# PKU-EPIC/GraspNeRF

Hardware: AMD Instinct MI355X
Metric: scenes/sec TSDF+render fwd, 6-view 40^3 grid (higher is better)
Workload: dtype f32

## Files before the change

graspnerf_amd/_lib.py:

```python
import ctypes as C
import os

_HERE = os.path.dirname(os.path.abspath(__file__))
LIB_PATH = os.path.join(_HERE, 'csrc', os.environ.get('GNR_LIB', 'libgnr.so'))

GNR_OK, GNR_ERR_ARG, GNR_ERR_SHAPE, GNR_ERR_HIP, GNR_ERR_WORKSPACE = 0, -1, -2, -3, -4
ERRORS = {-1: 'GNR_ERR_ARG', -2: 'GNR_ERR_SHAPE', -3: 'GNR_ERR_HIP', -4: 'GNR_ERR_WORKSPACE'}

c_float_p = C.POINTER(C.c_float)


class GnrScene(C.Structure):
    _fields_ = [('B', C.c_int), ('V', C.c_int), ('H', C.c_int), ('W', C.c_int), ('fh', C.c_int), ('fw', C.c_int),
                ('imgs', C.c_void_p), ('img_feats', C.c_void_p), ('ray_feats', C.c_void_p),
                ('poses', C.c_void_p), ('Ks', C.c_void_p), ('depth_range', C.c_void_p), ('use_vis', C.c_int), ('options', C.c_uint)]


OPTIONS = {'fp32_chain': 0x001, 'feature_grad_fixed': 0x002, 'view1_one_wavefront': 0x004, 'view2_one_wavefront': 0x008,
           'ray_order_morton': 0x010, 'poison_partials': 0x020, 'direct_scatter': 0x040, 'geo_dual_fp32': 0x080, 'test_lose_partner': 0x100, 'static_tiles': 0x200, 'split_launch': 0x400}
GNR_STATUS_LOST_PARTNER = 16


class GnrRays(C.Structure):
    _fields_ = [('rn', C.c_int), ('dn', C.c_int), ('fdn', C.c_int),
                ('ray_mask_view_num', C.c_int), ('ray_mask_point_num', C.c_int),
                ('coords', C.c_void_p), ('que_pose', C.c_void_p), ('que_K', C.c_void_p),
                ('que_depth_range', C.c_void_p), ('que_imgs', C.c_void_p), ('fine_u', C.c_void_p),
                ('ray_batch_num', C.c_int), ('fine_depth_use_all', C.c_int)]


RENDER_OUT_FIELDS = ['depth', 'sdf_values', 'alpha_values', 'colors_nr', 'hit_prob_nr', 'pixel_colors_nr',
                     'pixel_colors_gt', 'render_depth', 'ray_mask', 'sdf_gradient_error', 'sdf_gradient', 'view_mask']


class GnrRenderOut(C.Structure):
    _fields_ = [(k, C.c_void_p) for k in RENDER_OUT_FIELDS]


GNR_GAUSS_MAX_RADIUS = 16


class GnrSelectParams(C.Structure):
    _fields_ = [('gauss_radius', C.c_int), ('gauss_w', C.c_double * (GNR_GAUSS_MAX_RADIUS + 1)),
                ('tsdf_thres_high', C.c_float), ('tsdf_thres_low', C.c_float), ('min_width', C.c_float),
                ('max_width', C.c_float), ('threshold', C.c_float), ('dilate_iterations', C.c_int),
                ('max_filter_size', C.c_int)]


class GnrError(RuntimeError):
    pass


# ... 1 lines not shown


def lib():
    global _lib
    if _lib is not None:
        return _lib
    if not os.path.exists(LIB_PATH):
        raise GnrError(f'{LIB_PATH} not found: build it with graspnerf_amd/csrc/build.sh '
                       f'(or __graft_entry__.build()); there is no CPU fallback for the hot path')
    import torch
    L = C.CDLL(LIB_PATH)
    L.gnr_canonical_weights_floats.restype = C.c_int
    L.gnr_packed_weights_floats.restype = C.c_int
    L.gnr_pack_weights.argtypes = [c_float_p, c_float_p]
    L.gnr_pack_weights.restype = C.c_int
    L.gnr_pack_vis_decoder.argtypes = [c_float_p, c_float_p]
    L.gnr_pack_vis_decoder.restype = C.c_int
    L.gnr_pack_vis_decoder_bwd.argtypes = [c_float_p, c_float_p]
    L.gnr_pack_vis_decoder_bwd.restype = C.c_int
    L.gnr_canonical_vis_floats.restype = C.c_int
    for name in ('gnr_pack_weights_device', 'gnr_pack_weights_bwd_device', 'gnr_pack_vis_decoder_device', 'gnr_pack_vis_decoder_bwd_device'):
        getattr(L, name).argtypes = [C.c_void_p, C.c_void_p, C.c_void_p]
        getattr(L, name).restype = C.c_int
    L.gnr_layout_offset.argtypes = [C.c_char_p]
    L.gnr_layout_offset.restype = C.c_int
    L.gnr_workspace_bytes.argtypes = [C.POINTER(GnrScene), C.c_int, C.c_int, C.c_int]
    L.gnr_workspace_bytes.restype = C.c_size_t
    L.gnr_prepare.argtypes = [C.POINTER(GnrScene), C.c_void_p, C.c_size_t, C.c_void_p]
    L.gnr_prepare.restype = C.c_int
    L.gnr_range_status.argtypes = [C.POINTER(GnrScene), C.c_void_p, C.c_size_t, C.POINTER(C.c_uint), C.c_void_p]
    L.gnr_range_status.restype = C.c_int
    L.gnr_status_words_offset.argtypes = [C.POINTER(GnrScene)]
    L.gnr_status_words_offset.restype = C.c_size_t
    L.gnr_sample_volume_fwd.argtypes = [C.POINTER(GnrScene), C.c_void_p, C.c_int, C.c_void_p, C.c_void_p,
                                        C.c_void_p, C.c_void_p, C.c_size_t, C.c_void_p]
    L.gnr_sample_volume_fwd.restype = C.c_int
    L.gnr_debug_volume_chain.argtypes = [C.POINTER(GnrScene), C.c_void_p, C.c_int, C.c_void_p, C.c_void_p,
                                         C.c_void_p, C.c_size_t, C.c_void_p]
    L.gnr_debug_volume_chain.restype = C.c_int
    L.gnr_depth_mean_fwd.argtypes = [C.POINTER(GnrScene), C.c_void_p, C.c_int, C.c_void_p, C.c_void_p,
                                     C.c_void_p, C.c_size_t, C.c_void_p]
    L.gnr_depth_mean_fwd.restype = C.c_int
    L.gnr_merge_depths.argtypes = [C.c_void_p, C.c_int, C.c_void_p, C.c_int, C.c_void_p, C.c_int, C.c_void_p]
    L.gnr_merge_depths.restype = C.c_int
    L.gnr_render_by_depth_fwd.argtypes = [C.POINTER(GnrScene), C.POINTER(GnrRays), C.c_void_p, C.c_int, C.c_void_p,
                                          C.POINTER(GnrRenderOut), C.c_void_p, C.c_size_t, C.c_void_p]
    L.gnr_render_by_depth_fwd.restype = C.c_int
    L.gnr_render_rays_fwd.argtypes = [C.POINTER(GnrScene), C.POINTER(GnrRays), C.c_void_p, C.c_void_p,
                                      C.POINTER(GnrRenderOut), C.POINTER(GnrRenderOut), C.c_void_p, C.c_void_p,
                                      C.c_void_p, C.c_size_t, C.c_void_p]
    L.gnr_render_rays_fwd.restype = C.c_int
    L.gnr_head_canonical_floats.restype = C.c_int
    L.gnr_head_packed_floats.restype = C.c_int
    L.gnr_pack_grasp_head.argtypes = [c_float_p, c_float_p]
    L.gnr_pack_grasp_head.restype = C.c_int
    L.gnr_grasp_head_workspace_bytes.argtypes = [C.c_int, C.c_int]
    L.gnr_grasp_head_workspace_bytes.restype = C.c_size_t
    L.gnr_grasp_head_fwd.argtypes = [C.c_int, C.c_int, C.c_void_p, C.c_void_p, C.c_void_p, C.c_void_p, C.c_void_p,
                                     C.c_void_p, C.c_size_t, C.c_void_p]
    L.gnr_grasp_head_fwd.restype = C.c_int
    L.gnr_head_last_error.restype = C.c_char_p
    L.gnr_conv3d_bwd_weight.argtypes = [C.c_void_p] * 3 + [C.c_int] * 7 + [C.c_void_p]
    L.gnr_conv3d_same_bwd_weight.argtypes = [C.c_void_p] * 3 + [C.c_int] * 7 + [C.c_void_p, C.c_size_t, C.c_void_p]
    L.gnr_conv3d_same_bwd_weight_workspace_bytes.argtypes = [C.c_int] * 7
    L.gnr_conv3d_same_bwd_weight_workspace_bytes.restype = C.c_size_t
    L.gnr_conv3d_same_bwd_weight.restype = C.c_int
# ... 65 lines not shown
                                      [C.c_void_p] * 6 + [C.c_int, C.c_void_p, C.c_size_t, C.c_void_p]
    L.gnr_grasp_select_fwd.restype = C.c_int
    L.gnr_post_last_error.restype = C.c_char_p
    L.gnr_time_chain_kernel.argtypes = [C.POINTER(GnrScene), C.c_int, C.c_void_p, C.c_void_p, C.c_size_t, C.c_int,
                                        c_float_p, C.c_void_p]
    L.gnr_time_chain_kernel.restype = C.c_int
    L.gnr_chain_timing_begin.restype = C.c_int
    L.gnr_timing_begin.restype = C.c_int
    L.gnr_timing_begin_only.argtypes = [C.c_char_p]
    L.gnr_timing_begin_only.restype = C.c_int
    L.gnr_timing_end.argtypes = [C.c_char_p, C.c_size_t]
    L.gnr_timing_end.restype = C.c_int
    L.gnr_chain_timing_end.argtypes = [c_float_p, C.POINTER(C.c_int)]
    L.gnr_chain_timing_end.restype = C.c_int
    L.gnr_img_last_error.restype = C.c_char_p
    L.gnr_instnorm_act.argtypes = [C.c_void_p] * 7 + [C.c_longlong, C.c_int, C.c_int, C.c_float, C.c_int, C.c_void_p]
    L.gnr_instnorm_act.restype = C.c_int
    L.gnr_instnorm_act_bwd.argtypes = [C.c_void_p] * 12 + [C.c_longlong, C.c_int, C.c_int, C.c_int, C.c_void_p]
    L.gnr_instnorm_act_bwd.restype = C.c_int
    for fn in (L.gnr_reflect_pad2d, L.gnr_reflect_pad2d_bwd):
        fn.argtypes = [C.c_void_p, C.c_void_p, C.c_longlong, C.c_int, C.c_int, C.c_int, C.c_void_p]
        fn.restype = C.c_int
    L.gnr_upsample2x_bilinear.argtypes = [C.c_void_p, C.c_void_p, C.c_longlong, C.c_int, C.c_int, C.c_void_p]
    L.gnr_upsample2x_bilinear.restype = C.c_int
    L.gnr_last_error.restype = C.c_char_p
    L.gnr_dominant_kernel_name.restype = C.c_char_p
    L.gnr_debug_fill_lds.argtypes = [C.c_uint, C.c_void_p]
    L.gnr_debug_fill_lds.restype = C.c_int
    _lib = L
    return L


EXPORTED = ['gnr_canonical_weights_floats', 'gnr_packed_weights_floats', 'gnr_pack_weights', 'gnr_pack_vis_decoder', 'gnr_pack_vis_decoder_bwd', 'gnr_canonical_vis_floats', 'gnr_pack_weights_device', 'gnr_pack_weights_bwd_device', 'gnr_pack_vis_decoder_device', 'gnr_pack_vis_decoder_bwd_device', 'gnr_layout_offset', 'gnr_workspace_bytes',
            'gnr_prepare', 'gnr_range_status', 'gnr_status_words_offset', 'gnr_sample_volume_fwd', 'gnr_debug_volume_chain', 'gnr_depth_mean_fwd', 'gnr_merge_depths', 'gnr_render_by_depth_fwd', 'gnr_render_rays_fwd',
            'gnr_dominant_kernel_name', 'gnr_last_error', 'gnr_time_chain_kernel', 'gnr_head_canonical_floats',
            'gnr_head_packed_floats', 'gnr_pack_grasp_head', 'gnr_grasp_head_workspace_bytes', 'gnr_grasp_head_fwd',
            'gnr_head_last_error', 'gnr_chain_timing_begin', 'gnr_chain_timing_end', 'gnr_timing_begin', 'gnr_timing_begin_only', 'gnr_timing_end', 'gnr_grasp_select_workspace_bytes',
            'gnr_grasp_select_fwd', 'gnr_post_last_error', 'gnr_packed_bwd_floats', 'gnr_pack_weights_bwd',
            'gnr_depth_mean_bwd_workspace_bytes', 'gnr_depth_mean_bwd', 'gnr_sample_volume_train_workspace_bytes',
            'gnr_train_workspace_layout', 'gnr_sample_volume_fwd_train', 'gnr_sample_volume_bwd',
            'gnr_render_chain_train_workspace_bytes', 'gnr_render_chain_fwd_train', 'gnr_render_chain_bwd', 'gnr_conv3d_bwd_weight', 'gnr_conv3d_same_workspace_bytes', 'gnr_conv3d_same', 'gnr_conv3d_tap_mask_words', 'gnr_conv3d_tap_mask', 'gnr_conv3d_same_masked', 'gnr_conv3d_same_bwd_weight_masked', 'gnr_conv3d_same_bwd_weight', 'gnr_conv3d_same_bwd_weight_workspace_bytes',
            'gnr_render_tail_fwd_train', 'gnr_ray_tail_grad_floats', 'gnr_ray_tail_dual_bwd', 'gnr_ray_tail_dual_bwd_workspace_bytes', 'gnr_composite_bwd', 'gnr_composite_bwd_workspace_bytes', 'gnr_geo_dual_fwd', 'gnr_geo_dual_fwd_workspace_bytes', 'gnr_geo_dual_bwd', 'gnr_geo_dual_bwd_workspace_bytes', 'gnr_host_randperm_prefix',
            'gnr_debug_fill_lds', 'gnr_img_last_error', 'gnr_instnorm_act', 'gnr_instnorm_act_bwd', 'gnr_reflect_pad2d', 'gnr_reflect_pad2d_bwd', 'gnr_upsample2x_bilinear']


def check(rc, what):
    if rc != GNR_OK:
        msg = lib().gnr_last_error().decode(errors='replace')
        raise GnrError(f'{what} failed: {ERRORS.get(rc, rc)} ({msg})')


def timing_begin(only=None):
    check(lib().gnr_timing_begin_only(only.encode() if only else None), 'gnr_timing_begin')


def timing_end():
    buf = C.create_string_buffer(1 << 16)
    n = lib().gnr_timing_end(buf, len(buf))
    if n < 0:
        check(n, 'gnr_timing_end')
    out = {}
    for line in buf.value.decode().splitlines():
        label, cnt, ms = line.rsplit(' ', 2)
        out[label] = (int(cnt), float(ms))
    return out
```

graspnerf_amd/csrc/gnr_capi.inc:

```
#include <stdio.h>
#include <string.h>
#include <atomic>
#include <mutex>

#include "../../include/gnr.h"

namespace gnr {

static thread_local char g_err[512] = "";
static int fail(int code, const char* what, hipError_t e = hipSuccess) {
    snprintf(g_err, sizeof(g_err), "%s%s%s", what, e != hipSuccess ? ": " : "", e != hipSuccess ? hipGetErrorString(e) : "");
    return code;
}
#define GNR_HIP(call)                                                         \
    do {                                                                      \
        hipError_t e_ = (call);                                               \
        if (e_ != hipSuccess) return fail(GNR_ERR_HIP, #call, e_);            \
    } while (0)

static inline size_t al256(size_t x) { return (x + 255) & ~(size_t)255; }

static bool attr_needed(std::atomic<unsigned long long>& done) {
    int dev = 0;
    if (hipGetDevice(&dev) != hipSuccess) return true;
    const unsigned long long bit = 1ull << (dev & 63);
    if (done.load() & bit) return false;
    done.fetch_or(bit);
    return true;
}

struct Workspace {
    float* feat64; float* viewp; unsigned* range_flag;
    float* desc; float* rec; float* depth_c; float* depth_f; float* depth_m; float* gerr_part; unsigned char* vmask_pts;
    int* ray_perm;
    size_t total;
};

static Workspace carve(const GnrScene* s, size_t P, size_t rn, void* base) {
    Workspace w;
    char* p = (char*)base;
    size_t off = 0;
    const size_t BV = (size_t)s->B * s->V;
    auto take = [&](size_t bytes) { char* q = p ? p + off : nullptr; off += al256(bytes); return q; };
    w.feat64 = (float*)take(BV * s->fh * s->fw * 64 * sizeof(float));
    w.viewp = (float*)take(BV * VIEWP_FLOATS * sizeof(float));
    w.range_flag = (unsigned*)take(512);
    w.desc = (float*)take((size_t)s->B * P * DESC_FLOATS * sizeof(float));
    w.rec = (float*)take((size_t)s->B * P * REC_RAY * sizeof(float));
    w.depth_c = (float*)take((size_t)s->B * P * sizeof(float));
    w.depth_f = (float*)take((size_t)s->B * P * sizeof(float));
    w.depth_m = (float*)take((size_t)s->B * P * sizeof(float));
    w.gerr_part = (float*)take((size_t)s->B * (rn > 0 ? rn : 1) * sizeof(float));
    w.vmask_pts = (unsigned char*)take((size_t)s->B * P);
    w.ray_perm = (int*)take((size_t)s->B * (rn > 0 ? rn : 1) * sizeof(int));
    w.total = off;
    return w;
}

enum StatusSlot { RS_SCENE = 0, RS_VOLUME = 1, RS_COARSE = 2, RS_FINE = 3, RS_VOLUME_TRAIN = 4, RS_COARSE_TRAIN = 5, RS_DEPTHS_TRAIN = 6,
                  RS_BACKWARD = 61 , RS_RAY_WATCH = 62 ,
                  RS_FEAT_FX = 63 , RS_WORDS = 64 };
static_assert(RS_DEPTHS_TRAIN < RS_BACKWARD && RS_FEAT_FX < RS_WORDS, "status slots");
static inline bool opt(const GnrScene* s, unsigned bit) { return (s->options & bit) != 0; }

static int check_scene(const GnrScene* s) {
    if (!s || !s->imgs || !s->img_feats || !s->ray_feats || !s->poses || !s->Ks || !s->depth_range)
        return fail(GNR_ERR_ARG, "GnrScene: null pointer");
    if (s->options & ~GNR_OPT_ALL) return fail(GNR_ERR_ARG, "GnrScene.options: unknown bits (GNR_OPT_*)");
    if (s->B < 1 || s->H < 2 || s->W < 2 || s->fh < 1 || s->fw < 1) return fail(GNR_ERR_SHAPE, "GnrScene: bad dims");
    if (s->V < 2 || s->V > 8) return fail(GNR_ERR_SHAPE, "GnrScene: V must be in 2..8");
    return GNR_OK;
}

static int check_points(const GnrScene* s, size_t P) {
    if ((size_t)s->B * P > ((size_t)1 << 31) - 1024) return fail(GNR_ERR_SHAPE, "too many points in one call (B*P must stay below 2^31): split the rays / scenes");
    return GNR_OK;
}

static bool brick_order_ok(int R) { return R % 8 == 0; }

static int num_cus() {
    static int n = 0;
    if (!n) {
        hipDeviceProp_t prop;
        int dev = 0;
        if (hipGetDevice(&dev) != hipSuccess || hipGetDeviceProperties(&prop, dev) != hipSuccess) return 256;
        n = prop.multiProcessorCount > 0 ? prop.multiProcessorCount : 256;
// ... 315 lines not shown
    if (int rc = check_scene(s)) return rc;
    if (!ws) return fail(GNR_ERR_ARG, "workspace is null");
    Workspace w = carve(s, 0, 0, ws);
    if (ws_bytes < w.total) return fail(GNR_ERR_WORKSPACE, "workspace too small");
    hipStream_t st = (hipStream_t)stream;
    const int npix = s->fh * s->fw, BV = s->B * s->V;
    { KScope ks("k_view_setup@gnr_prepare", st); hipLaunchKernelGGL(k_view_setup, dim3((BV + 63) / 64), dim3(64), 0, st, s->poses, s->Ks, s->depth_range, w.viewp, BV, w.range_flag); }
    GNR_HIP(hipGetLastError());
    { KScope ks("k_repack_feats@gnr_prepare", st); hipLaunchKernelGGL(k_repack_feats, dim3((npix + 63) / 64, BV), dim3(256), 0, st, s->ray_feats, s->img_feats, w.feat64, npix, w.range_flag); }
    GNR_HIP(hipGetLastError());
    return GNR_OK;
}

extern "C" int gnr_range_status(const GnrScene* s, const void* ws, size_t ws_bytes, unsigned* flags_out, void* stream) {
    if (int rc = check_scene(s)) return rc;
    if (!ws || !flags_out) return fail(GNR_ERR_ARG, "gnr_range_status: null pointer");
    Workspace w = carve(s, 0, 0, const_cast<void*>(ws));
    if (ws_bytes < w.total) return fail(GNR_ERR_WORKSPACE, "workspace too small");
    hipStream_t st = (hipStream_t)stream;
    unsigned words[RS_WORDS];
    GNR_HIP(hipMemcpyAsync(words, w.range_flag, sizeof(words), hipMemcpyDeviceToHost, st));
    GNR_HIP(hipStreamSynchronize(st));
    unsigned f = 0;
    for (int i = 0; i < RS_WORDS; ++i) f |= words[i];
    *flags_out = f;
    return GNR_OK;
}

extern "C" size_t gnr_status_words_offset(const GnrScene* s) {
    if (!s) return 0;
    char* const base = (char*)4096;
    Workspace w = carve(s, 0, 0, base);
    return (size_t)((char*)w.range_flag - base);
}

struct SideStream { hipStream_t st = nullptr; hipEvent_t fork = nullptr, join = nullptr; };
static SideStream* side_stream() {
    static SideStream tab[64];
    static std::atomic<unsigned long long> made{0};
    int dev = 0;
    if (hipGetDevice(&dev) != hipSuccess) return nullptr;
    SideStream& e = tab[dev & 63];
    const unsigned long long bit = 1ull << (dev & 63);
    if (!(made.load() & bit)) {
        static std::mutex mu;
        std::lock_guard<std::mutex> lk(mu);
        if (!(made.load() & bit)) {
            if (hipStreamCreateWithFlags(&e.st, hipStreamNonBlocking) != hipSuccess) return nullptr;
            if (hipEventCreateWithFlags(&e.fork, hipEventDisableTiming) != hipSuccess || hipEventCreateWithFlags(&e.join, hipEventDisableTiming) != hipSuccess) return nullptr;
            made.fetch_or(bit);
        }
    }
    return &e;
}

static int volume_impl(const GnrScene* s, const float* bbox_min, int R, const float* wc, float* sdf_out,
                       unsigned char* vmask_out, void* ws, size_t ws_bytes, hipStream_t st, bool points, bool chain, bool ray,
                       float* dbg = nullptr) {
    if (int rc = check_points(s, (size_t)R * R * R)) return rc;
    Workspace w = carve(s, (size_t)R * R * R, 0, ws);
    if (ws_bytes < w.total) return fail(GNR_ERR_WORKSPACE, "workspace too small");
    const int P = R * R * R;
    const bool inline_pts = GNR_VOLUME_POINTS_INLINE != 0 && chain && ray && !dbg && R * R * R < (1 << 22);
    if (points && !inline_pts) {
        { KScope ks("k_points_volume@volume_impl", st); hipLaunchKernelGGL(k_points_volume, dim3((s->B * P + 255) / 256), dim3(256), 0, st, bbox_min, w.desc, R, s->B); }
        GNR_HIP(hipGetLastError());
// ... 25 lines not shown
            if (int rc = launch_ray<false>(r, ps)) return rc;
        }
    }
    if (split) { GNR_HIP(hipEventRecord(side->join, side->st)); GNR_HIP(hipStreamWaitEvent(st, side->join, 0)); }
    return GNR_OK;
}

extern "C" int gnr_sample_volume_fwd(const GnrScene* s, const float* bbox_min, int R, const float* wc, float* sdf_out,
                                     unsigned char* vmask_out, void* ws, size_t ws_bytes, void* stream) {
    if (int rc = check_scene(s)) return rc;
    if (!bbox_min || !wc || !sdf_out || !ws) return fail(GNR_ERR_ARG, "gnr_sample_volume_fwd: null pointer");
    if (R < 2 || R > MAX_DN) return fail(GNR_ERR_SHAPE, "volume_res must be in 2..64");
    return volume_impl(s, bbox_min, R, wc, sdf_out, vmask_out, ws, ws_bytes, (hipStream_t)stream, true, true, true);
}

extern "C" int gnr_debug_volume_chain(const GnrScene* s, const float* bbox_min, int R, const float* wc, float* dbg,
                                      void* ws, size_t ws_bytes, void* stream) {
    if (int rc = check_scene(s)) return rc;
    if (!bbox_min || !wc || !dbg || !ws) return fail(GNR_ERR_ARG, "gnr_debug_volume_chain: null pointer");
    return volume_impl(s, bbox_min, R, wc, nullptr, nullptr, ws, ws_bytes, (hipStream_t)stream, true, true, false, dbg);
}

static int order_rays(const GnrScene* s, const GnrRays* q, Workspace& w, hipStream_t st, const int** perm_out) {
    *perm_out = nullptr;
    if (!opt(s, GNR_OPT_RAY_ORDER_MORTON) || q->rn > MAX_SORT_RAYS || q->rn < 2) return GNR_OK;
    int shift = 0;
    while (((s->W > s->H ? s->W : s->H) >> shift) > 1024) ++shift;
    { KScope ks("k_ray_order@render_pass", st); hipLaunchKernelGGL(k_ray_order, dim3(s->B), dim3(256), 0, st, q->coords, w.ray_perm, q->rn, shift); }
    GNR_HIP(hipGetLastError());
    *perm_out = w.ray_perm;
    return GNR_OK;
}

static int render_pass(const GnrScene* s, const GnrRays* q, const float* depth, int dn, const float* wl, GnrRenderOut* out,
                       Workspace& w, hipStream_t st, float* fine_depth, int* fine_inds, int fdn, const float* fine_u = nullptr,
                       const int* perm = nullptr, int range_slot = RS_COARSE, float* gt_also = nullptr, bool skip_gt = false, bool gen_depth = false) {
    if (!out || !out->colors_nr) return fail(GNR_ERR_ARG, "GnrRenderOut.colors_nr is required");
    const int B = s->B, rn = q->rn;
    const int P = rn * dn;
    { KScope ks("k_points_rays@render_pass", st); hipLaunchKernelGGL(k_points_rays, dim3((B * P + 255) / 256), dim3(256), 0, st, q->coords, q->que_pose, q->que_K,
                       q->que_depth_range, depth, w.desc, rn, dn, B, perm, gen_depth ? const_cast<float*>(depth) : nullptr); }
    GNR_HIP(hipGetLastError());
    ChainArgs a{wl, w.feat64, s->imgs, w.viewp, w.desc, w.rec, out->colors_nr, out->view_mask, nullptr,
                B, P, s->H, s->W, s->fh, s->fw, 0};
    a.range_flag = w.range_flag;
    a.range_launch = w.range_flag ? w.range_flag + range_slot : nullptr;
    a.tile_ctr = (w.range_flag && !opt(s, GNR_OPT_STATIC_TILES)) ? w.range_flag + RS_WORDS : nullptr;
    a.ray_perm = perm; a.perm_rn = rn; a.perm_dn = dn;
    if (int rc = launch_chain<true>(s, a, st)) return rc;
    RayArgs r;
    memset(&r, 0, sizeof(r));
    r.wpk = wl; r.rec = w.rec; r.desc = w.desc; r.depth = depth; r.colors = out->colors_nr; r.que_dr = q->que_depth_range;
    r.nrays = B * rn; r.dn = dn; r.rays_per_scene = rn;
    r.sdf = out->sdf_values; r.alpha = out->alpha_values; r.hit = out->hit_prob_nr; r.pix = out->pixel_colors_nr;
    r.rdepth = out->render_depth; r.gerr_part = out->sdf_gradient_error ? w.gerr_part : nullptr; r.grad = out->sdf_gradient;
    r.rmask = out->ray_mask; r.view_num = q->ray_mask_view_num; r.point_num = q->ray_mask_point_num;
    r.fine_depth = fine_depth; r.fine_inds = fine_inds; r.fdn = fdn; r.fine_u = fine_u; r.ray_perm = perm;
    r.range_word = w.range_flag ? w.range_flag + RS_RAY_WATCH : nullptr;
    if (int rc = launch_ray<true>(r, st)) return rc;
    if (out->sdf_gradient_error) {
        const int chunk = q->ray_batch_num > 0 ? q->ray_batch_num : rn;
        { KScope ks("k_gerr_reduce@render_pass", st); hipLaunchKernelGGL(k_gerr_reduce, dim3(B, (rn + chunk - 1) / chunk), dim3(256), 0, st, w.gerr_part,
                           out->sdf_gradient_error, rn, dn, chunk); }
        GNR_HIP(hipGetLastError());
    }
    if (out->pixel_colors_gt && q->que_imgs && !skip_gt) {
        { KScope ks("k_pixel_gt@render_pass", st); hipLaunchKernelGGL(k_pixel_gt, dim3((B * rn + 255) / 256), dim3(256), 0, st, q->que_imgs, q->coords, out->pixel_colors_gt,
                           rn, s->H, s->W, B, gt_also); }
        GNR_HIP(hipGetLastError());
    }
    if (out->depth && out->depth != depth)
        GNR_HIP(hipMemcpyAsync(out->depth, depth, (size_t)B * P * sizeof(float), hipMemcpyDeviceToDevice, st));
    return GNR_OK;
}

static int check_rays(const GnrRays* q, bool by_depth = false) {
    if (!q || !q->coords || !q->que_pose || !q->que_K || !q->que_depth_range) return fail(GNR_ERR_ARG, "GnrRays: null pointer");
    if (q->rn < 1) return fail(GNR_ERR_SHAPE, "GnrRays: rn must be positive");
    if (!by_depth && (q->dn < 3 || q->dn > MAX_DN || q->fdn < 1 || q->fdn > MAX_DN)) return fail(GNR_ERR_SHAPE, "GnrRays: dn/fdn must be in 3..64");
    if (q->fine_depth_use_all != 0 && q->fine_depth_use_all != 1) return fail(GNR_ERR_ARG, "GnrRays: fine_depth_use_all must be 0 or 1");
    if (q->ray_batch_num < 0) return fail(GNR_ERR_SHAPE, "GnrRays: ray_batch_num must be >= 0");
// ... 797 lines not shown
```

graspnerf_amd/csrc/gnr_kernels.hip:

```cpp
#include <hip/hip_runtime.h>
#include <stdint.h>
#include <type_traits>

#include "gnr_layout.h"

#ifndef GNR_ABLATE
#define GNR_ABLATE 0
#endif

namespace gnr {

typedef float f4 __attribute__((ext_vector_type(4)));
typedef float f2 __attribute__((ext_vector_type(2)));

#define DEV __device__ __forceinline__

DEV f4 mfma16(float a, float b, f4 c) { return __builtin_amdgcn_mfma_f32_16x16x4f32(a, b, c, 0, 0, 0); }
DEV float elu1(float x) { return fmaxf(x, __builtin_amdgcn_fmed3f(__expf(x), 0.f, 1.f) - 1.f); }
constexpr float kLog2e = 1.4426950408889634f, kLn2 = 0.6931471805599453f;
#if GNR_ABLATE & 8
DEV float elu_s(float xs) { return xs; }
#else
DEV float elu_s(float xs) { return fmaxf(xs, fmaf(__builtin_amdgcn_fmed3f(__builtin_amdgcn_exp2f(xs), 0.f, 1.f), kLog2e, -kLog2e)); }
#endif
// ... 435 lines not shown

__global__ void k_desc_unpack(const float* __restrict__ desc, float* __restrict__ pts, float* __restrict__ qdir, int dn, int n) {
    const int i = blockIdx.x * blockDim.x + threadIdx.x;
    if (i >= n) return;
    const float* d = desc + (size_t)i * DESC_FLOATS;
    if (pts) { pts[(size_t)i * 3] = d[0]; pts[(size_t)i * 3 + 1] = d[1]; pts[(size_t)i * 3 + 2] = d[2]; }
    if (qdir && i % dn == 0) { float* q = qdir + (size_t)(i / dn) * 3; q[0] = d[3]; q[1] = d[4]; q[2] = d[5]; }
}

struct ChainArgs {
    const float* wpk;
    const float* feat64;
    const float* imgs;
    const float* viewp;
    const float* desc;
    float* rec;
    float* colors;
    unsigned char* vmask;
    float* dbg;
    int B, P, H, W, fh, fw;
    int vol_res;
    float* save1;
    float* save2;
    float* saveG;
    float* saveZ;
    unsigned* range_flag;
    int only_if_flagged;
    unsigned* range_launch;
    const int* ray_perm; int perm_rn, perm_dn;
    unsigned* tile_ctr;
    const float* bbox_min;
    int pts_R;
    int b0;
};

struct ViewGeom {
    float u, v, z, m;
    float dd[4];
};

template <bool FULL>
DEV void project_view(const float* __restrict__ vp, const float (&p)[3], const float (&qd)[3], int H, int W, ViewGeom& o) {
    const float pcx = __fmaf_rn(vp[2], p[2], __fmaf_rn(vp[1], p[1], __fmul_rn(vp[0], p[0]))) + vp[3];
    const float pcy = __fmaf_rn(vp[6], p[2], __fmaf_rn(vp[5], p[1], __fmul_rn(vp[4], p[0]))) + vp[7];
    float z = __fmaf_rn(vp[10], p[2], __fmaf_rn(vp[9], p[1], __fmul_rn(vp[8], p[0]))) + vp[11];
    const bool inval = fabsf(z) < 1e-4f;
    if (inval) z = 1e-3f;
    o.z = z;
    o.u = __fdiv_rn(pcx, z);
    o.v = __fdiv_rn(pcy, z);
    const bool outside = (o.u < -0.5f) | (o.u >= (float)W - 0.5f) | (o.v < -0.5f) | (o.v >= (float)H - 0.5f);
    o.m = (!inval && !outside) ? 1.f : 0.f;
    if constexpr (FULL) {
        float d[3] = {p[0] - vp[12], p[1] - vp[13], p[2] - vp[14]};
        const float inr = -__builtin_amdgcn_rsqf(fmaxf(d[0] * d[0] + d[1] * d[1] + d[2] * d[2], 1e-10f));
        d[0] *= inr; d[1] *= inr; d[2] *= inr;
        o.dd[0] = d[0] - qd[0]; o.dd[1] = d[1] - qd[1]; o.dd[2] = d[2] - qd[2];
        o.dd[3] = d[0] * qd[0] + d[1] * qd[1] + d[2] * qd[2];
    }
}

struct Taps { int o00, o01, o10, o11; float w00, w01, w10, w11; };
DEV Taps make_taps(float u, float v, float sx, float sy, float off, int fh, int fw) {
    float px = fmaf(u, sx, off), py = fmaf(v, sy, off);
    px = fminf(fmaxf(px, 0.f), (float)(fw - 1));
    py = fminf(fmaxf(py, 0.f), (float)(fh - 1));
// ... 25 lines not shown
    const int stride = __float_as_int(ci.x), n1 = __float_as_int(ci.y);
    const bool outside = (q < -0.5f) | (q >= c.w);
    float px = fmaf(q, c.x, c.y);
    px = fminf(fmaxf(px, 0.f), c.z);
    const float x0 = floorf(px);
    const float w1 = px - x0;
    const int i0 = (int)x0, i1 = min(i0 + 1, n1);
    const int o0 = __mul24(i0, stride), o1 = __mul24(i1, stride);
    const int w1b = __float_as_int(w1) | ((outside | inval) ? (int)0x80000000 : 0);
    int O0[4], O1[4], W1[4];
#pragma unroll
    for (int k = 0; k < 4; ++k) {
        O0[k] = __builtin_amdgcn_ds_bpermute(bp + 64 * k, o0);
        O1[k] = __builtin_amdgcn_ds_bpermute(bp + 64 * k, o1);
        W1[k] = __builtin_amdgcn_ds_bpermute(bp + 64 * k, w1b);
    }
    o.m = ((W1[0] | W1[1]) >= 0) ? 1.f : 0.f;
    auto assemble = [&](int kx, int ky, Taps& t) {
        t.o00 = O0[ky] + O0[kx]; t.o01 = O0[ky] + O1[kx]; t.o10 = O1[ky] + O0[kx]; t.o11 = O1[ky] + O1[kx];
        const float wx1 = fabsf(__int_as_float(W1[kx])), wy1 = fabsf(__int_as_float(W1[ky])), wx0 = 1.f - wx1, wy0 = 1.f - wy1;
        t.w00 = wx0 * wy0; t.w01 = wx1 * wy0; t.w10 = wx0 * wy1; t.w11 = wx1 * wy1;
    };
    assemble(0, 1, o.f);
    assemble(2, 3, o.i);
}
DEV void view_dir(const float* __restrict__ vp, const float (&p)[3], const float (&qd)[3], float (&dd)[4]) {
    float d[3] = {p[0] - vp[12], p[1] - vp[13], p[2] - vp[14]};
    const float inr = -__builtin_amdgcn_rsqf(fmaxf(d[0] * d[0] + d[1] * d[1] + d[2] * d[2], 1e-10f));
    d[0] *= inr; d[1] *= inr; d[2] *= inr;
    dd[0] = d[0] - qd[0]; dd[1] = d[1] - qd[1]; dd[2] = d[2] - qd[2];
    dd[3] = d[0] * qd[0] + d[1] * qd[1] + d[2] * qd[2];
}

constexpr int SW = 20;
#ifndef GNR_TWO_QUEUES
#define GNR_TWO_QUEUES 0
#endif
#ifndef GNR_RDF2_PAIRS
#define GNR_RDF2_PAIRS 0
#endif
constexpr int rows_a(int V) { return GNR_TWO_QUEUES ? (V + 1) / 2 : V; }
constexpr int rows_b(int V) { return GNR_TWO_QUEUES ? V / 2 : 0; }

#ifndef GNR_DYN_TILES
#define GNR_DYN_TILES 1
#endif
#ifndef GNR_VOLUME_POINTS_INLINE
#define GNR_VOLUME_POINTS_INLINE 1
#endif
#ifndef GNR_TAIL_OLD_ONLY
#define GNR_TAIL_OLD_ONLY 0
#endif
#ifndef GNR_DESC_PREFETCH
#define GNR_DESC_PREFETCH 0
#endif
#ifndef GNR_DYN_CTR_INC
#define GNR_DYN_CTR_INC 0
#endif
#ifndef GNR_DYN_TRAIN
#define GNR_DYN_TRAIN 1
#endif
#ifndef GNR_SKIP_MASKED
#define GNR_SKIP_MASKED 1
#endif
#ifndef GNR_CHAIN_THREADS
#define GNR_CHAIN_THREADS 512
// ... 80 lines not shown
    const bool dyn = GNR_DYN_TILES != 0 && (GNR_DYN_TRAIN > 1 || !(SAVE && RENDER)) && (GNR_DYN_TRAIN != 0 || !SAVE) && a.tile_ctr != nullptr;
    int cx = xcd;
#if GNR_DYN_CTR_INC
    auto grab = [&]() -> unsigned { unsigned t = 0u; if (lane == 0) t = atomicInc(a.tile_ctr + cx, 0xFFFFFFFFu); return t; };
#else
    auto grab = [&]() -> unsigned { unsigned t = 0u; if (lane == 0) t = atomicAdd(a.tile_ctr + cx, 1u); return t; };
#endif
    auto resolve = [&](unsigned t_raw) -> int {
        int t = __builtin_amdgcn_readfirstlane((int)t_raw);
#if GNR_DYN_TILES > 1
        for (int hops = 0; t >= min(ntiles, (cx + 1) * chunk) - cx * chunk;) {
            if (++hops >= NXCD) return -1;
            cx = cx + 1 == NXCD ? 0 : cx + 1;
            t = __builtin_amdgcn_readfirstlane((int)grab());
        }
        return cx * chunk + t;
#else
        return t < t_end - xcd * chunk ? xcd * chunk + t : -1;
#endif
    };
    auto locate = [&](int tile_, int& b_, int& ts_) {
        b_ = tile_ / tps;
        ts_ = tile_ - b_ * tps;
        b_ += a.b0;
        if (a.vol_res > 0) {
            const int R = a.vol_res, tpg = R >> 3, gpr = R >> 1;
            const int BX = R >> 2, GY = R >> 3, GB = BX * GY;
            const int sidx = ts_ / tpg, tin = ts_ - sidx * tpg;
            const int brick = sidx / GB, wi = sidx - brick * GB;
            const int bx = brick >> 2, by = brick & 3;
            ts_ = ((BX * bx + wi / GY) * gpr + GY * by + wi % GY) * tpg + tin;
        }
    };
    auto point_of = [&](int b_, int ts_) -> size_t { const int nr = ts_ * 16 + r; return (size_t)b_ * a.P + (nr < a.P ? nr : a.P - 1); };
    int tile = dyn ? resolve(grab()) : xcd * chunk + lblk * waves_per_block + wave;
    constexpr bool DPF = GNR_DESC_PREFETCH != 0 && !SAVE;
    f4 d0n = {0.f, 0.f, 0.f, 0.f}, d1n = d0n;
    bool have_nxt = false;
    for (; dyn ? tile >= 0 : tile < t_end;) {
        GNR_ITER_FENCE();
        unsigned tile_nxt = 0u;
        int tile_after = -1;
#if GNR_WAVE_CLOCK
        const unsigned long long wc_tt = wall_clock64();
#endif
        int b, ts;
        locate(tile, b, ts);
        const int n_raw = ts * 16 + r;
        const bool row_ok = n_raw < a.P;
        const int n = row_ok ? n_raw : a.P - 1;
        const size_t pt = (size_t)b * a.P + n;
        size_t opt = pt;
        if (RENDER && !SAVE && a.ray_perm) {
            const int s_ = n / a.perm_dn;
            opt = (size_t)b * a.P + (size_t)a.ray_perm[(size_t)b * a.perm_rn + s_] * a.perm_dn + (n - s_ * a.perm_dn);
        }
        float p[3], qd[3], lo, hi;
        {
            f4 d0, d1;
            if (DPF && have_nxt) { d0 = d0n; d1 = d1n; }
            else if (!RENDER && !SAVE && GNR_VOLUME_POINTS_INLINE != 0 && a.pts_R > 0) {
                const int R = a.pts_R;
                const float invR = 1.f / (float)R;
                const int col = (int)(((float)n + 0.5f) * invR), sz = n - col * R;
                const int ix = (int)(((float)col + 0.5f) * invR), iy = col - ix * R, iz = R - 1 - sz;
                const double vs = 0.3 / (double)R, hv = vs / 2;
                const float* bm = a.bbox_min + b * 3;
                d0 = (f4){(float)(ix * vs + hv) + bm[0], (float)(iy * vs + hv) + bm[1], (float)(iz * vs + hv) + bm[2], 0.f};
                d1 = (f4){0.f, 1.f, 0.005f, 0.005f};
            }
            else { d0 = reinterpret_cast<const f4*>(a.desc)[pt * 2]; d1 = reinterpret_cast<const f4*>(a.desc)[pt * 2 + 1]; }
            p[0] = d0.x; p[1] = d0.y; p[2] = d0.z; qd[0] = d0.w; qd[1] = d1.x; qd[2] = d1.y; lo = d1.z; hi = d1.w;
        }
        constexpr int VA = rows_a(V), VB = rows_b(V);
        float SA[VA][SW], SB[VB > 0 ? VB : 1][SW];
        auto S = [&](int v, int q) -> float& { return (VB == 0 || v < VA) ? SA[v < VA ? v : 0][q] : SB[v >= VA ? v - VA : 0][q]; };
#pragma unroll
        for (int k = 0; k < V; ++k)
#pragma unroll
#if GNR_ABLATE & 1
            for (int q = 0; q < SW; ++q) S(k, q) = p[0] * (float)(k * SW + q + 1);
#else
            for (int q = 0; q < SW; ++q) S(k, q) = 0.f;
// ... 1226 lines not shown
```

include/gnr.h:

```cpp
#ifndef GNR_H
#define GNR_H
#include <stddef.h>

#ifdef __cplusplus
extern "C" {
#endif

#define GNR_OK 0
#define GNR_ERR_ARG (-1)
#define GNR_ERR_SHAPE (-2)
#define GNR_ERR_HIP (-3)
#define GNR_ERR_WORKSPACE (-4)

typedef struct GnrScene {
    int B, V;
    int H, W;
    int fh, fw;
    const float* imgs;
    const float* img_feats;
    const float* ray_feats;
    const float* poses;
    const float* Ks;
    const float* depth_range;
    int use_vis;
    unsigned options;
} GnrScene;

#define GNR_OPT_FP32_CHAIN 0x001u
#define GNR_OPT_FEATURE_GRAD_FIXED 0x002u
#define GNR_OPT_VIEW1_ONE_WAVEFRONT 0x004u
#define GNR_OPT_VIEW2_ONE_WAVEFRONT 0x008u
#define GNR_OPT_RAY_ORDER_MORTON 0x010u
#define GNR_OPT_POISON_PARTIALS 0x020u
#define GNR_OPT_DIRECT_SCATTER 0x040u
#define GNR_OPT_GEO_DUAL_FP32 0x080u
#define GNR_OPT_TEST_LOSE_PARTNER 0x100u
#define GNR_OPT_STATIC_TILES 0x200u
#define GNR_OPT_SPLIT_LAUNCH 0x400u
#define GNR_OPT_ALL 0x7ffu

typedef struct GnrRays {
    int rn;
    int dn;
    int fdn;
    int ray_mask_view_num;
    int ray_mask_point_num;
    const float* coords;
    const float* que_pose;
    const float* que_K;
    const float* que_depth_range;
    const float* que_imgs;
    const float* fine_u;
    int ray_batch_num;
    int fine_depth_use_all;
} GnrRays;

typedef struct GnrRenderOut {
    float* depth;
    float* sdf_values;
    float* alpha_values;
    float* colors_nr;
    float* hit_prob_nr;
    float* pixel_colors_nr;
    float* pixel_colors_gt;
    float* render_depth;
    unsigned char* ray_mask;
    float* sdf_gradient_error;
    float* sdf_gradient;
    unsigned char* view_mask;
} GnrRenderOut;

int gnr_canonical_weights_floats(void);
int gnr_packed_weights_floats(void);
int gnr_pack_weights(const float* canonical_host, float* packed_host);
int gnr_pack_vis_decoder(const float* vis_decoder_host, float* packed_host);
int gnr_pack_vis_decoder_bwd(const float* vis_decoder_host, float* packed_bwd_host);
int gnr_canonical_vis_floats(void);
int gnr_pack_weights_device(const float* canonical_dev, float* packed_dev, void* stream);
int gnr_pack_weights_bwd_device(const float* canonical_dev, float* packed_bwd_dev, void* stream);
int gnr_pack_vis_decoder_device(const float* vis_decoder_dev, float* packed_dev, void* stream);
int gnr_pack_vis_decoder_bwd_device(const float* vis_decoder_dev, float* packed_bwd_dev, void* stream);
int gnr_layout_offset(const char* name);

size_t gnr_workspace_bytes(const GnrScene* scene, int volume_res, int rn, int dn_max);

int gnr_prepare(const GnrScene* scene, void* workspace, size_t workspace_bytes, void* stream);

#define GNR_STATUS_LOST_PARTNER 16u
int gnr_range_status(const GnrScene* scene, const void* workspace, size_t workspace_bytes, unsigned* flags_out, void* stream);
size_t gnr_status_words_offset(const GnrScene* scene);

int gnr_sample_volume_fwd(const GnrScene* scene, const float* bbox_min , int volume_res,
                          const float* packed_coarse , float* sdf_out ,
                          unsigned char* view_mask_out, void* workspace, size_t workspace_bytes,
                          void* stream);

int gnr_render_by_depth_fwd(const GnrScene* scene, const GnrRays* rays, const float* depth, int dn,
                            const float* level_weights, GnrRenderOut* out, void* workspace,
                            size_t workspace_bytes, void* stream);

int gnr_render_rays_fwd(const GnrScene* scene, const GnrRays* rays, const float* packed_coarse,
                        const float* packed_fine, GnrRenderOut* coarse, GnrRenderOut* fine,
                        const float* fine_depth_in, int* fine_inds_out, void* workspace,
                        size_t workspace_bytes, void* stream);

int gnr_merge_depths(const float* depth_a, int na, const float* depth_b, int nb, float* out, int nrays, void* stream);

int gnr_depth_mean_fwd(const GnrScene* scene, const float* coords, int pn, const float* level_weights,
                       float* mean_out, void* workspace, size_t workspace_bytes, void* stream);

int gnr_debug_volume_chain(const GnrScene* scene, const float* bbox_min, int volume_res,
                           const float* packed_coarse, float* dbg, void* workspace,
                           size_t workspace_bytes, void* stream);

int gnr_head_canonical_floats(void);
int gnr_head_packed_floats(void);
int gnr_pack_grasp_head(const float* canonical_host, float* packed_host);
size_t gnr_grasp_head_workspace_bytes(int B, int volume_res);
int gnr_grasp_head_fwd(int B, int volume_res, const float* volume, const float* packed_head, float* qual, float* rot,
                       float* width, void* workspace, size_t workspace_bytes, void* stream);
const char* gnr_head_last_error(void);
int gnr_conv3d_bwd_weight(const float* x, const float* dy, float* dw, int B, int Cin, int Cout, int D, int H, int W, int K,
                          void* stream);
// ... 111 lines not shown
```

Baseline: 4916.

## Sort render samples by view-visibility mask before running the chain kernel

Adds a two-kernel counting sort that computes a per-sample visibility bitmask over the views, builds per-chunk histograms, and writes a permutation that groups samples by mask, ordered by visible-view count. The render chain kernel then reads samples through this permutation, so wavefronts handle samples with the same visibility and diverge less. This costs two extra launches, a projection of every sample per view, and indirect gathers of descriptors. It can be turned off with a new option bit.

```diff
diff --git a/graspnerf_amd/_lib.py b/graspnerf_amd/_lib.py
--- a/graspnerf_amd/_lib.py
+++ b/graspnerf_amd/_lib.py
@@ -17,7 +17,8 @@
 
 
 OPTIONS = {'fp32_chain': 0x001, 'feature_grad_fixed': 0x002, 'view1_one_wavefront': 0x004, 'view2_one_wavefront': 0x008,
-           'ray_order_morton': 0x010, 'poison_partials': 0x020, 'direct_scatter': 0x040, 'geo_dual_fp32': 0x080, 'test_lose_partner': 0x100, 'static_tiles': 0x200, 'split_launch': 0x400}
+           'ray_order_morton': 0x010, 'poison_partials': 0x020, 'direct_scatter': 0x040, 'geo_dual_fp32': 0x080, 'test_lose_partner': 0x100, 'static_tiles': 0x200, 'split_launch': 0x400,
+           'sample_order_off': 0x800}
 GNR_STATUS_LOST_PARTNER = 16
 
 
@@ -85,6 +86,8 @@
     L.gnr_range_status.restype = C.c_int
     L.gnr_status_words_offset.argtypes = [C.POINTER(GnrScene)]
     L.gnr_status_words_offset.restype = C.c_size_t
+    L.gnr_sample_order_offset.argtypes = [C.POINTER(GnrScene), C.c_int, C.c_int]
+    L.gnr_sample_order_offset.restype = C.c_size_t
     L.gnr_sample_volume_fwd.argtypes = [C.POINTER(GnrScene), C.c_void_p, C.c_int, C.c_void_p, C.c_void_p,
                                         C.c_void_p, C.c_void_p, C.c_size_t, C.c_void_p]
     L.gnr_sample_volume_fwd.restype = C.c_int
@@ -216,7 +219,7 @@
 
 
 EXPORTED = ['gnr_canonical_weights_floats', 'gnr_packed_weights_floats', 'gnr_pack_weights', 'gnr_pack_vis_decoder', 'gnr_pack_vis_decoder_bwd', 'gnr_canonical_vis_floats', 'gnr_pack_weights_device', 'gnr_pack_weights_bwd_device', 'gnr_pack_vis_decoder_device', 'gnr_pack_vis_decoder_bwd_device', 'gnr_layout_offset', 'gnr_workspace_bytes',
-            'gnr_prepare', 'gnr_range_status', 'gnr_status_words_offset', 'gnr_sample_volume_fwd', 'gnr_debug_volume_chain', 'gnr_depth_mean_fwd', 'gnr_merge_depths', 'gnr_render_by_depth_fwd', 'gnr_render_rays_fwd',
+            'gnr_prepare', 'gnr_range_status', 'gnr_status_words_offset', 'gnr_sample_order_offset', 'gnr_sample_volume_fwd', 'gnr_debug_volume_chain', 'gnr_depth_mean_fwd', 'gnr_merge_depths', 'gnr_render_by_depth_fwd', 'gnr_render_rays_fwd',
             'gnr_dominant_kernel_name', 'gnr_last_error', 'gnr_time_chain_kernel', 'gnr_head_canonical_floats',
             'gnr_head_packed_floats', 'gnr_pack_grasp_head', 'gnr_grasp_head_workspace_bytes', 'gnr_grasp_head_fwd',
             'gnr_head_last_error', 'gnr_chain_timing_begin', 'gnr_chain_timing_end', 'gnr_timing_begin', 'gnr_timing_begin_only', 'gnr_timing_end', 'gnr_grasp_select_workspace_bytes',
diff --git a/graspnerf_amd/csrc/gnr_capi.inc b/graspnerf_amd/csrc/gnr_capi.inc
--- a/graspnerf_amd/csrc/gnr_capi.inc
+++ b/graspnerf_amd/csrc/gnr_capi.inc
@@ -33,6 +33,7 @@
     float* feat64; float* viewp; unsigned* range_flag;
     float* desc; float* rec; float* depth_c; float* depth_f; float* depth_m; float* gerr_part; unsigned char* vmask_pts;
     int* ray_perm;
+    int* pt_order; unsigned char* pt_keys; int* pt_hist;
     size_t total;
 };
 
@@ -53,6 +54,9 @@
     w.gerr_part = (float*)take((size_t)s->B * (rn > 0 ? rn : 1) * sizeof(float));
     w.vmask_pts = (unsigned char*)take((size_t)s->B * P);
     w.ray_perm = (int*)take((size_t)s->B * (rn > 0 ? rn : 1) * sizeof(int));
+    w.pt_order = (int*)take((size_t)s->B * P * sizeof(int));
+    w.pt_keys = (unsigned char*)take((size_t)s->B * P);
+    w.pt_hist = (int*)take((size_t)s->B * ((P + ORDER_CHUNK - 1) / ORDER_CHUNK) * 256 * sizeof(int));
     w.total = off;
     return w;
 }
@@ -434,6 +438,13 @@
     char* const base = (char*)4096;
     Workspace w = carve(s, 0, 0, base);
     return (size_t)((char*)w.range_flag - base);
+}
+
+extern "C" size_t gnr_sample_order_offset(const GnrScene* s, int rn, int dn_max) {
+    if (!s || rn < 0 || dn_max < 0) return 0;
+    char* const base = (char*)4096;
+    Workspace w = carve(s, (size_t)rn * dn_max, rn, base);
+    return (size_t)((char*)w.pt_order - base);
 }
 
 struct SideStream { hipStream_t st = nullptr; hipEvent_t fork = nullptr, join = nullptr; };
@@ -525,6 +536,19 @@
     return GNR_OK;
 }
 
+static int order_samples(const GnrScene* s, int P, Workspace& w, hipStream_t st, const int** order_out) {
+    *order_out = nullptr;
+    if (opt(s, GNR_OPT_SAMPLE_ORDER_OFF)) return GNR_OK;
+    const int chunks = (P + ORDER_CHUNK - 1) / ORDER_CHUNK;
+    const unsigned blocks = (unsigned)((size_t)s->B * chunks);
+    { KScope ks("k_sample_keys@render_pass", st); hipLaunchKernelGGL(k_sample_keys, dim3(blocks), dim3(256), 0, st, w.desc, w.viewp, w.pt_keys, w.pt_hist, P, s->V, s->H, s->W, chunks); }
+    GNR_HIP(hipGetLastError());
+    { KScope ks("k_sample_order@render_pass", st); hipLaunchKernelGGL(k_sample_order, dim3(blocks), dim3(64), 0, st, w.pt_keys, w.pt_hist, w.pt_order, P, s->V, chunks); }
+    GNR_HIP(hipGetLastError());
+    *order_out = w.pt_order;
+    return GNR_OK;
+}
+
 static int render_pass(const GnrScene* s, const GnrRays* q, const float* depth, int dn, const float* wl, GnrRenderOut* out,
                        Workspace& w, hipStream_t st, float* fine_depth, int* fine_inds, int fdn, const float* fine_u = nullptr,
                        const int* perm = nullptr, int range_slot = RS_COARSE, float* gt_also = nullptr, bool skip_gt = false, bool gen_depth = false) {
@@ -540,6 +564,7 @@
     a.range_launch = w.range_flag ? w.range_flag + range_slot : nullptr;
     a.tile_ctr = (w.range_flag && !opt(s, GNR_OPT_STATIC_TILES)) ? w.range_flag + RS_WORDS : nullptr;
     a.ray_perm = perm; a.perm_rn = rn; a.perm_dn = dn;
+    if (int rc = order_samples(s, P, w, st, &a.pt_order)) return rc;
     if (int rc = launch_chain<true>(s, a, st)) return rc;
     RayArgs r;
     memset(&r, 0, sizeof(r));
diff --git a/graspnerf_amd/csrc/gnr_kernels.hip b/graspnerf_amd/csrc/gnr_kernels.hip
--- a/graspnerf_amd/csrc/gnr_kernels.hip
+++ b/graspnerf_amd/csrc/gnr_kernels.hip
@@ -491,6 +491,7 @@
     const float* bbox_min;
     int pts_R;
     int b0;
+    const int* pt_order;
 };
 
 struct ViewGeom {
@@ -582,6 +583,95 @@
     dd[3] = d[0] * qd[0] + d[1] * qd[1] + d[2] * qd[2];
 }
 
+constexpr int ORDER_CHUNK = 1024;
+__global__ __launch_bounds__(256) void k_sample_keys(const float* __restrict__ desc, const float* __restrict__ viewp, unsigned char* __restrict__ keys,
+                                                     int* __restrict__ hist, int P, int V, int H, int W, int chunks) {
+    constexpr int PER = ORDER_CHUNK / 256;
+    __shared__ int cnt[256];
+    const int b = blockIdx.x / chunks, c = blockIdx.x - b * chunks, NP = 1 << V;
+    for (int k = threadIdx.x; k < NP; k += 256) cnt[k] = 0;
+    float p[PER][3];
+#pragma unroll
+    for (int j = 0; j < PER; ++j) {
+        const int n = min(c * ORDER_CHUNK + j * 256 + (int)threadIdx.x, P - 1);
+        const f4 d0 = reinterpret_cast<const f4*>(desc)[((size_t)b * P + n) * 2];
+        p[j][0] = d0.x; p[j][1] = d0.y; p[j][2] = d0.z;
+    }
+    const float qd[3] = {0.f, 0.f, 0.f};
+    unsigned bits[PER];
+#pragma unroll
+    for (int j = 0; j < PER; ++j) bits[j] = 0u;
+    for (int v = 0; v < V; ++v) {
+        const float* vp = viewp + ((size_t)b * V + v) * VIEWP_FLOATS;
+#pragma unroll
+        for (int j = 0; j < PER; ++j) {
+            ViewGeom vg;
+            project_view<false>(vp, p[j], qd, H, W, vg);
+            bits[j] |= (vg.m != 0.f ? 1u : 0u) << v;
+        }
+    }
+    __syncthreads();
+#pragma unroll
+    for (int j = 0; j < PER; ++j) {
+        const int n = c * ORDER_CHUNK + j * 256 + (int)threadIdx.x;
+        if (n < P) {
+            keys[(size_t)b * P + n] = (unsigned char)bits[j];
+            atomicAdd(&cnt[bits[j]], 1);
+        }
+    }
+    __syncthreads();
+    int* h = hist + (size_t)blockIdx.x * 256;
+    for (int k = threadIdx.x; k < NP; k += 256) h[k] = cnt[k];
+}
+
+__global__ __launch_bounds__(64) void k_sample_order(const unsigned char* __restrict__ keys, const int* __restrict__ hist, int* __restrict__ order,
+                                                     int P, int V, int chunks) {
+    constexpr int ROUNDS = ORDER_CHUNK / 64;
+    __shared__ int tot[256], base[256];
+    const int b = blockIdx.x / chunks, c = blockIdx.x - b * chunks, NP = 1 << V, lane = threadIdx.x;
+    const int n0 = c * ORDER_CHUNK, n1 = min(P, n0 + ORDER_CHUNK);
+    unsigned key[ROUNDS];
+#pragma unroll
+    for (int j = 0; j < ROUNDS; ++j) { const int n = n0 + j * 64 + lane; key[j] = n < n1 ? keys[(size_t)b * P + n] : 0u; }
+    const int* h = hist + (size_t)b * chunks * 256;
+    for (int k = lane; k < NP; k += 64) {
+        int t = 0, pre = 0;
+        for (int c0 = 0; c0 < chunks; c0 += 8) {
+            int x[8];
+#pragma unroll
+            for (int j = 0; j < 8; ++j) x[j] = c0 + j < chunks ? h[(size_t)(c0 + j) * 256 + k] : 0;
+#pragma unroll
+            for (int j = 0; j < 8; ++j) { t += x[j]; pre += c0 + j < c ? x[j] : 0; }
+        }
+        tot[k] = t; base[k] = pre;
+    }
+    __syncthreads();
+    for (int k = lane; k < NP; k += 64) {
+        const int ck = __popc(k);
+        int s = 0;
+#pragma unroll 8
+        for (int q = 0; q < NP; ++q) { const int cq = __popc(q); s += (cq > ck || (cq == ck && q < k)) ? tot[q] : 0; }
+        base[k] += s;
+    }
+    __syncthreads();
+    const unsigned long long below = (1ull << lane) - 1ull;
+#pragma unroll
+    for (int j = 0; j < ROUNDS; ++j) {
+        const int n = n0 + j * 64 + lane;
+        const bool ok = n < n1;
+        unsigned long long same = __ballot(ok);
+        for (int i = 0; i < V; ++i) {
+            const bool bit = ((key[j] >> i) & 1u) != 0u;
+            const unsigned long long on = __ballot(ok && bit);
+            same &= bit ? on : ~on;
+        }
+        if (ok) {
+            order[(size_t)b * P + base[key[j]] + __popcll(same & below)] = n;
+            if ((same & below) == 0ull) base[key[j]] += __popcll(same);
+        }
+    }
+}
+
 constexpr int SW = 20;
 #ifndef GNR_TWO_QUEUES
 #define GNR_TWO_QUEUES 0
@@ -728,7 +818,8 @@
             ts_ = ((BX * bx + wi / GY) * gpr + GY * by + wi % GY) * tpg + tin;
         }
     };
-    auto point_of = [&](int b_, int ts_) -> size_t { const int nr = ts_ * 16 + r; return (size_t)b_ * a.P + (nr < a.P ? nr : a.P - 1); };
+    auto in_order = [&](int b_, int n_) -> int { return (RENDER && !SAVE && a.pt_order) ? a.pt_order[(size_t)b_ * a.P + n_] : n_; };
+    auto point_of = [&](int b_, int ts_) -> size_t { const int nr = ts_ * 16 + r; return (size_t)b_ * a.P + in_order(b_, nr < a.P ? nr : a.P - 1); };
     int tile = dyn ? resolve(grab()) : xcd * chunk + lblk * waves_per_block + wave;
     constexpr bool DPF = GNR_DESC_PREFETCH != 0 && !SAVE;
     f4 d0n = {0.f, 0.f, 0.f, 0.f}, d1n = d0n;
@@ -744,7 +835,7 @@
         locate(tile, b, ts);
         const int n_raw = ts * 16 + r;
         const bool row_ok = n_raw < a.P;
-        const int n = row_ok ? n_raw : a.P - 1;
+        const int n = in_order(b, row_ok ? n_raw : a.P - 1);
         const size_t pt = (size_t)b * a.P + n;
         size_t opt = pt;
         if (RENDER && !SAVE && a.ray_perm) {
diff --git a/include/gnr.h b/include/gnr.h
--- a/include/gnr.h
+++ b/include/gnr.h
@@ -37,7 +37,8 @@
 #define GNR_OPT_TEST_LOSE_PARTNER 0x100u
 #define GNR_OPT_STATIC_TILES 0x200u
 #define GNR_OPT_SPLIT_LAUNCH 0x400u
-#define GNR_OPT_ALL 0x7ffu
+#define GNR_OPT_SAMPLE_ORDER_OFF 0x800u
+#define GNR_OPT_ALL 0xfffu
 
 typedef struct GnrRays {
     int rn;
@@ -89,6 +90,7 @@
 #define GNR_STATUS_LOST_PARTNER 16u
 int gnr_range_status(const GnrScene* scene, const void* workspace, size_t workspace_bytes, unsigned* flags_out, void* stream);
 size_t gnr_status_words_offset(const GnrScene* scene);
+size_t gnr_sample_order_offset(const GnrScene* scene, int rn, int dn_max);
 
 int gnr_sample_volume_fwd(const GnrScene* scene, const float* bbox_min , int volume_res,
                           const float* packed_coarse , float* sdf_out ,
```

New measurement: 5001 (median of 6 runs). 1.7% higher.
